# Sbte/RAILS

Measured on AMD Instinct MI355X. Metric: RAILS iterations/sec (+ A*V SpMM HBM GB/s in roofline), m=1M rows/GPU, k=128, fp64, higher is better.
Workload: dtype f64

## Files before the change

### include/rails_hip.h

```cpp
#ifndef RAILS_HIP_H
#define RAILS_HIP_H

#include <stddef.h>
#include <stdint.h>

#ifdef __cplusplus
extern "C" {
#endif

#define RAILS_OK 0
#define RAILS_EINVAL -1
#define RAILS_EHIP -2
#define RAILS_ENOMEM -3
#define RAILS_ELAPACK -4
#define RAILS_ECOMM -5
#define RAILS_ENODEV -6

typedef struct rails_ctx rails_ctx;
typedef struct rails_csr rails_csr;
typedef struct rails_panel rails_panel;

const char *rails_last_error(void);
const char *rails_version(void);


int rails_ctx_create(int device, void *stream, rails_ctx **out);
int rails_ctx_destroy(rails_ctx *ctx);
int rails_ctx_sync(rails_ctx *ctx);
void *rails_ctx_stream(rails_ctx *ctx);
int rails_ctx_stats(rails_ctx *ctx, char *buf, int cap);
int rails_ctx_set_meter(rails_ctx *ctx, int on);

int rails_ctx_set_seed(rails_ctx *ctx, uint64_t seed, uint64_t first_stream);
int rails_ctx_rng_state(rails_ctx *ctx, uint64_t *seed, uint64_t *next_stream);

int rails_ctx_set_partition(rails_ctx *ctx, int rank, int nranks, int64_t row0, int64_t m_global);

typedef int (*rails_allreduce_fn)(void *user, double *dev_buf, size_t n, void *stream);
int rails_ctx_set_allreduce(rails_ctx *ctx, rails_allreduce_fn fn, void *user);

#define RAILS_RCCL_ID_BYTES 128
int rails_rccl_unique_id(void *id_out);
int rails_ctx_init_rccl(rails_ctx *ctx, const void *id, int nranks, int rank);
int rails_ctx_set_rccl(rails_ctx *ctx, void *nccl_comm);
int rails_ctx_rccl_size(const rails_ctx *ctx);

typedef int (*rails_halo_fn)(void *user, const double *send_buf, double *recv_buf, int ncols, void *stream);


// ... 56 lines not shown
int rails_panel_reserve(rails_ctx *ctx, rails_panel *P, int capacity);

int rails_panel_upload(rails_ctx *ctx, rails_panel *P, int c0, int nc, const double *host, int64_t ldh);
int rails_panel_download(rails_ctx *ctx, const rails_panel *P, int c0, int nc, double *host, int64_t ldh);

int rails_panel_fill(rails_ctx *ctx, rails_panel *P, int c0, int nc, double value);
int rails_panel_scale(rails_ctx *ctx, rails_panel *P, int c0, int nc, double s);
int rails_panel_copy(rails_ctx *ctx, const rails_panel *X, int xc0, int nc, rails_panel *Y, int yc0);
int rails_panel_axpy(rails_ctx *ctx, double alpha, const rails_panel *X, int xc0, int nc, rails_panel *Y,
                     int yc0);
int rails_panel_random(rails_ctx *ctx, rails_panel *P, int c0, int nc);

int rails_gram(rails_ctx *ctx, const rails_panel *X, int xc0, int a, const rails_panel *Y, int yc0, int b,
               double *C_host, int ldc);

int rails_panel_gemm(rails_ctx *ctx, double alpha, const rails_panel *X, int xc0, int k, const double *C_host,
                     int ldc, int r, double beta, rails_panel *Y, int yc0);

int rails_ctx_enable_library_gemm(rails_ctx *ctx);
int rails_ctx_library_gemm_ready(const rails_ctx *ctx);

int rails_deferred_reserve(rails_ctx *ctx, int nslots, int64_t doubles_per_slot);
int rails_gram_deferred(rails_ctx *ctx, const rails_panel *X, int xc0, int a, const rails_panel *Y, int yc0, int b, int slot);
int rails_panel_gemm_deferred(rails_ctx *ctx, double alpha, const rails_panel *X, int xc0, int k, int slot, int ld, int r, double beta,
                              rails_panel *Y, int yc0);
int rails_chol_inverse_deferred(rails_ctx *ctx, int slot_in, int w, int slot_out);
int rails_update_gram_deferred(rails_ctx *ctx, double alpha, const rails_panel *X, int xc0, int k, const double *C_host, int ldc, int r,
                               rails_panel *Y, int yc0, int r2, int slot);
int rails_deferred_fetch(rails_ctx *ctx, int slot, int64_t n, double *host_out);

int rails_panel_gemm_wide(rails_ctx *ctx, double alpha, const rails_panel *X, int xc0, int k, const double *C_host, int ldc, int r,
                          double beta, rails_panel *Y, int yc0);

int rails_orthogonalize(rails_ctx *ctx, rails_panel *V, int k_old, int w, int method, int *used);
int rails_orthogonalize_deflated(rails_ctx *ctx, rails_panel *V, int k_old, int w, const rails_panel *N, int nc0, int q, int method, int *used);

int rails_resid_lanczos(rails_ctx *ctx, const rails_panel *AV, int avc0, const rails_panel *MV, int mvc0, int k,
                        const double *T_host, int ldt, const rails_panel *B, int bc0, int p, int L,
                        double *H_host, int ldh, int *steps);

int rails_lanczos_start(rails_ctx *ctx, const rails_panel *AV, int avc0, const rails_panel *MV, int mvc0, int k,
                        const rails_panel *B, int bc0, int p, double *sums_host);

int rails_lanczos_vectors(rails_ctx *ctx, const double *S_host, int lds, int w, rails_panel *Out, int oc0);
int rails_lanczos_release(rails_ctx *ctx);

int rails_ctx_reserve_staging(rails_ctx *ctx, size_t bytes);
int rails_timer_start(rails_ctx *ctx);
int rails_timer_stop(rails_ctx *ctx, double *ms);


void rails_sb03md(char dico, char job, char fact, char trans, int n, double *A, int lda, double *X, int ldx,
                  double *scale, int *info);
void rails_sb03md_counts(long *smith, long *schur);
void rails_sb03md_adi_counts(long *extended, long *fresh);
void rails_sb03md_set_pause(int calls);
void rails_dsyev(char jobz, char uplo, int n, double *a, int lda, double *w, int *info);
void rails_dsteqr(char compz, int n, double *d, double *e, double *z, int ldz, double *work, int *info);
void rails_dgemm(char transa, char transb, int m, int n, int k, double alpha, const double *A, int lda, const double *B,
                 int ldb, double beta, double *C, int ldc);
void rails_dtrsm(char side, char uplo, char transa, char diag, int m, int n, double alpha, const double *A, int lda, double *B, int ldb);
void rails_dpotrf(char uplo, int n, double *a, int lda, int *info);
void rails_dpstrf(char uplo, int n, double *a, int lda, int *piv, int *rank, double tol, int *info);
void rails_range_basis(int m, int n, double *a, int lda, double tol, double *q, int ldq, int *rank, int *info);
int rails_host_lapack_init(const char *path);
const char *rails_host_lapack_path(void);

#ifdef __cplusplus
}
#endif
#endif
```

### rails_amd/_lib.py

```python
import ctypes as C
import os

_HERE = os.path.dirname(os.path.abspath(__file__))
LIB_PATH = os.path.join(_HERE, "lib", "librails_hip.so")

_dp = C.POINTER(C.c_double)
_ip = C.POINTER(C.c_int)
_i64p = C.POINTER(C.c_int64)
_i32p = C.POINTER(C.c_int32)
_vp = C.c_void_p

ALLREDUCE_FN = C.CFUNCTYPE(C.c_int, C.c_void_p, C.c_void_p, C.c_size_t, C.c_void_p)
HALO_FN = C.CFUNCTYPE(C.c_int, C.c_void_p, C.c_void_p, C.c_void_p, C.c_int, C.c_void_p)
APPLY_FN = C.CFUNCTYPE(C.c_int, C.c_void_p, C.c_int, C.c_void_p, C.c_int, C.c_int, C.c_void_p, C.c_int)

SIGNATURES = {
    "rails_last_error": (C.c_char_p, []),
    "rails_version": (C.c_char_p, []),
    "rails_ctx_create": (C.c_int, [C.c_int, _vp, C.POINTER(_vp)]),
    "rails_ctx_destroy": (C.c_int, [_vp]),
    "rails_ctx_sync": (C.c_int, [_vp]),
    "rails_ctx_stream": (_vp, [_vp]),
    "rails_ctx_set_meter": (C.c_int, [_vp, C.c_int]),
    "rails_ctx_enable_library_gemm": (C.c_int, [_vp]),
# ... 29 lines not shown
    "rails_sweep_plan_create": (C.c_int, [C.c_int64, C.c_int64, _i64p, _i32p, _dp, _ip, C.POINTER(_vp)]),
    "rails_sweep_plan_destroy": (C.c_int, [_vp]),
    "rails_sweep_plan_info": (C.c_int, [_vp, _i64p, _dp]),
    "rails_sweep_plan_array": (C.c_int, [_vp, C.c_int, C.POINTER(_vp), _i64p]),
    "rails_panel_create": (C.c_int, [_vp, C.c_int64, C.c_int, C.POINTER(_vp)]),
    "rails_panel_destroy": (C.c_int, [_vp]),
    "rails_panel_rows": (C.c_int64, [_vp]),
    "rails_panel_capacity": (C.c_int, [_vp]),
    "rails_panel_ld": (C.c_int, [_vp]),
    "rails_panel_device_ptr": (_vp, [_vp]),
    "rails_panel_reserve": (C.c_int, [_vp, _vp, C.c_int]),
    "rails_panel_upload": (C.c_int, [_vp, _vp, C.c_int, C.c_int, _dp, C.c_int64]),
    "rails_panel_download": (C.c_int, [_vp, _vp, C.c_int, C.c_int, _dp, C.c_int64]),
    "rails_panel_fill": (C.c_int, [_vp, _vp, C.c_int, C.c_int, C.c_double]),
    "rails_panel_scale": (C.c_int, [_vp, _vp, C.c_int, C.c_int, C.c_double]),
    "rails_panel_copy": (C.c_int, [_vp, _vp, C.c_int, C.c_int, _vp, C.c_int]),
    "rails_panel_axpy": (C.c_int, [_vp, C.c_double, _vp, C.c_int, C.c_int, _vp, C.c_int]),
    "rails_sptrsv_create": (C.c_int, [_vp, C.c_int64, _i64p, _i32p, _dp, C.c_int, C.c_int, C.POINTER(_vp)]),
    "rails_sptrsv_destroy": (None, [_vp]),
    "rails_sptrsv_levels": (C.c_int64, [_vp]),
    "rails_sptrsv_solve": (C.c_int, [_vp, _vp, _vp, C.c_int, C.c_int]),
    "rails_panel_permute_rows": (C.c_int, [_vp, _vp, C.c_int, C.c_int, _vp, C.c_int, _vp, C.c_int]),
    "rails_index_upload": (C.c_int, [_vp, _i32p, C.c_int64, C.POINTER(_vp)]),
    "rails_index_free": (None, [_vp, _vp]),
    "rails_lu_create": (C.c_int, [_vp, C.c_int64, _i64p, _i32p, _dp, _i64p, _i32p, _dp, _i32p, _i32p, _i32p, C.c_int64, C.POINTER(_vp)]),
    "rails_lu_destroy": (None, [_vp]),
    "rails_lu_solve": (C.c_int, [_vp, _vp, C.c_int, _vp, C.c_int, C.c_int, _vp, C.c_int]),
    "rails_lu_stats": (C.c_int, [_vp, _i64p, C.c_int]),
    "rails_csr_create_lu": (C.c_int, [_vp, _vp, C.POINTER(_vp)]),
    "rails_panel_random": (C.c_int, [_vp, _vp, C.c_int, C.c_int]),
    "rails_gram": (C.c_int, [_vp, _vp, C.c_int, C.c_int, _vp, C.c_int, C.c_int, _dp, C.c_int]),
    "rails_panel_gemm": (C.c_int, [_vp, C.c_double, _vp, C.c_int, C.c_int, _dp, C.c_int, C.c_int, C.c_double, _vp, C.c_int]),
    "rails_panel_gemm_wide": (C.c_int, [_vp, C.c_double, _vp, C.c_int, C.c_int, _dp, C.c_int, C.c_int, C.c_double, _vp, C.c_int]),
    "rails_orthogonalize": (C.c_int, [_vp, _vp, C.c_int, C.c_int, C.c_int, _ip]),
    "rails_orthogonalize_deflated": (C.c_int, [_vp, _vp, C.c_int, C.c_int, _vp, C.c_int, C.c_int, C.c_int, _ip]),
    "rails_resid_lanczos": (C.c_int, [_vp, _vp, C.c_int, _vp, C.c_int, C.c_int, _dp, C.c_int, _vp, C.c_int, C.c_int, C.c_int,
                                      _dp, C.c_int, _ip]),
    "rails_lanczos_start": (C.c_int, [_vp, _vp, C.c_int, _vp, C.c_int, C.c_int, _vp, C.c_int, C.c_int, _dp]),
    "rails_lanczos_vectors": (C.c_int, [_vp, _dp, C.c_int, C.c_int, _vp, C.c_int]),
    "rails_lanczos_release": (C.c_int, [_vp]),
    "rails_timer_start": (C.c_int, [_vp]),
    "rails_timer_stop": (C.c_int, [_vp, _dp]),
    "rails_sb03md": (None, [C.c_char, C.c_char, C.c_char, C.c_char, C.c_int, _dp, C.c_int, _dp, C.c_int, _dp, _ip]),
    "rails_dsyev": (None, [C.c_char, C.c_char, C.c_int, _dp, C.c_int, _dp, _ip]),
    "rails_dsteqr": (None, [C.c_char, C.c_int, _dp, _dp, _dp, C.c_int, _dp, _ip]),
    "rails_ctx_reserve_staging": (C.c_int, [_vp, C.c_size_t]),
    "rails_sb03md_set_pause": (None, [C.c_int]),
    "rails_sb03md_counts": (None, [C.POINTER(C.c_long), C.POINTER(C.c_long)]),
    "rails_sb03md_adi_counts": (None, [C.POINTER(C.c_long), C.POINTER(C.c_long)]),
    "rails_dtrsm": (None, [C.c_char, C.c_char, C.c_char, C.c_char, C.c_int, C.c_int, C.c_double, _dp, C.c_int, _dp, C.c_int]),
    "rails_dgemm": (None, [C.c_char, C.c_char, C.c_int, C.c_int, C.c_int, C.c_double, _dp, C.c_int, _dp, C.c_int, C.c_double, _dp, C.c_int]),
    "rails_dpotrf": (None, [C.c_char, C.c_int, _dp, C.c_int, _ip]),
    "rails_dpstrf": (None, [C.c_char, C.c_int, _dp, C.c_int, _ip, _ip, C.c_double, _ip]),
    "rails_range_basis": (None, [C.c_int, C.c_int, _dp, C.c_int, C.c_double, _dp, C.c_int, _ip, _ip]),
    "rails_host_lapack_init": (C.c_int, [C.c_char_p]),
    "rails_host_lapack_path": (C.c_char_p, []),
}

_lib = None


class RailsError(RuntimeError):
    pass


def load():
    global _lib
    if _lib is not None:
        return _lib
    if not os.path.exists(LIB_PATH):
        raise RailsError(
            "rails_amd: %s is missing -- build it with `python -c 'import __graft_entry__ as g; g.build()'` "
            "or `make -C rails_amd/csrc`; there is no CPU fallback" % LIB_PATH)
    lib = C.CDLL(LIB_PATH, mode=C.RTLD_GLOBAL)
    for name, (res, args) in SIGNATURES.items():
        fn = getattr(lib, name)
        fn.restype = res
        fn.argtypes = args
    try:
        from ._solver_sigs import bind as _bind_solver
        _bind_solver(lib)
    except ImportError:
        pass
    _lib = lib
    return lib


# ... 5 lines not shown
```

### rails_amd/csrc/host_numerics.cpp

```cpp
#include <dlfcn.h>

#include <algorithm>
#include <atomic>
#include <chrono>
#include <utility>
#include <cmath>
#include <cstdio>
#include <cstdlib>
#include <cstring>
#include <mutex>
#include <string>
#include <vector>

#include "rails_hip.h"

void rails_set_error(const char *fmt, ...);

namespace {

extern "C" {
typedef int (*lp_select2)(const double *, const double *);
typedef void (*lp_dsyev)(const char *, const char *, const int *, double *, const int *, double *, double *, const int *, int *);
typedef void (*lp_dsyevd)(const char *, const char *, const int *, double *, const int *, double *, double *, const int *, int *, const int *, int *);
typedef void (*lp_dsteqr)(const char *, const int *, double *, double *, double *, const int *, double *, int *);
// ... 315 lines not shown
    *rank = 0;
    if (rails_host_lapack_init(nullptr) != RAILS_OK || !g_lp.dgeqp3 || !g_lp.dorgqr) {
        *info = -100;
        return;
    }
    if (m <= 0 || n <= 0) {
        *info = 0;
        return;
    }
    const int kmin = m < n ? m : n;
    std::vector<int> jpvt((size_t)n, 0);
    std::vector<double> tau((size_t)kmin);
    double wq = 0.0;
    int lwork = -1;
    g_lp.dgeqp3(&m, &n, a, &lda, jpvt.data(), tau.data(), &wq, &lwork, info);
    if (*info != 0) return;
    lwork = (int)wq + 1;
    std::vector<double> work((size_t)lwork);
    g_lp.dgeqp3(&m, &n, a, &lda, jpvt.data(), tau.data(), work.data(), &lwork, info);
    if (*info != 0) return;
    const double r11 = std::fabs(a[0]);
    int r = 0;
    while (r < kmin && std::fabs(a[r + (size_t)r * lda]) > tol * r11 && r11 > 0.0) ++r;
    *rank = r;
    if (r == 0) return;
    for (int j = 0; j < r; ++j)
        for (int i = 0; i < m; ++i) q[i + (size_t)j * ldq] = a[i + (size_t)j * lda];
    lwork = -1;
    g_lp.dorgqr(&m, &r, &r, q, &ldq, tau.data(), &wq, &lwork, info);
    if (*info != 0) return;
    lwork = (int)wq + 1;
    work.resize((size_t)lwork);
    g_lp.dorgqr(&m, &r, &r, q, &ldq, tau.data(), work.data(), &lwork, info);
}

static int &sb03md_smith_pause()
{
    static thread_local int pause = 0;
    return pause;
}
static int &sb03md_factored_pause()
{
    static thread_local int pause = 0;
    return pause;
}
extern "C" void rails_sb03md_set_pause(int calls) { sb03md_smith_pause() = sb03md_factored_pause() = calls > 0 ? calls : 0; }
static std::atomic<long> g_sb03md_smith{0}, g_sb03md_schur{0};
extern "C" void rails_sb03md_counts(long *smith, long *schur)
{
    if (smith) *smith = g_sb03md_smith.load();
    if (schur) *schur = g_sb03md_schur.load();
}

static bool smith_lyapunov(bool tr, int n, const double *A, int lda, double *X, int ldx)
{
    if (!g_lp.dgetrf || !g_lp.dgetrs) return false;
    const size_t nn = (size_t)n * n;
    std::vector<double> M(nn), S(nn), Ak(nn), Y(nn), T1(nn), T2(nn), C(nn);
    double trace = 0.0;
    for (int j = 0; j < n; ++j) {
        for (int i = 0; i < n; ++i) {
            M[i + (size_t)j * n] = tr ? A[i + (size_t)j * lda] : A[j + (size_t)i * lda];
            C[i + (size_t)j * n] = 0.5 * (X[i + (size_t)j * ldx] + X[j + (size_t)i * ldx]);
        }
        trace += A[j + (size_t)j * lda];
    }
// ... 569 lines not shown
```

### rails_amd/csrc/solver_capi.cpp

```cpp
#include <cmath>
#include <cstdio>
#include <cstring>
#include <map>
#include <string>
#include <vector>

#include <exception>
#include <new>

#include "rails/HipSolverOps.hpp"
#include "rails/SubspaceSolverOps.hpp"
#include "rails_solver.h"

void rails_set_error(const char *fmt, ...);

namespace
{

class ParameterList
{
    std::map<std::string, double> params_;

public:
    template <typename T>
// ... 206 lines not shown
    rails::HipSolver::Projection proj;
    const bool pair = rails::HipSolver::parse_projection(s->params.get("Projection method", 1.0), proj) && proj.pair;
    const int kmax = std::max(restart > 0 ? restart : 100, 1) + (pair ? 2 : 1) * expand + 100;
    auto basis = std::make_shared<rails::SubspaceBasis>(s->ctx, s->m_local, s->m_global, 2 * kmax + p + 128);
    if (restart > 0 || s->params.get("Restart iterations", 20) > 0) basis->preallocate_compress_panel();
    rails::SubspaceMultiVector Bc = rails::SubspaceMultiVector::Absorb(basis, s->B);
    rails::SubspaceOperator Ac(s->A, basis);
    rails::SubspaceOperator Mc(s->mass ? s->M : s->A, basis);
    rails::SubspaceSolver solver(Ac, Bc, Mc);
    if (s->has_inv) solver.set_inverse(rails::SubspaceOperator(s->Ainv, basis));
    if (s->null_q > 0) solver.set_nullspace(rails::SubspaceMultiVector::Absorb(basis, s->N));
    int prc = solver.set_parameters(s->params);
    if (prc != 0) return prc + 100;
    solver.set_verbose(s->verbose);
    solver.set_max_trips(s->max_trips);
    solver.use_mass_matrix(s->mass);
    solver.use_mass_orthogonalisation(s->ortho_m);
    if (s->trip_fn) solver.set_trip_callback([s](int trip) { s->trip_fn(s->trip_user, trip); });
    solver.set_failure_check([basis]() { return basis->failed; });
    rails::SubspaceMultiVector Vc(basis, 1);
    if (s->have_V0) {
        Vc = rails::SubspaceMultiVector::Absorb(basis, s->V);
        Vc.set_orthogonalized(Vc.N());
    }
    int rc = solver.solve(Vc, s->T);
    s->null_rank = solver.nullspace_rank();
    if (rc == -2) return rc;
    s->V = Vc.materialise();
    s->V.set_orthogonalized(s->V.N());
    s->sub_trips = solver.trips();
    s->sub_hist = solver.residual_history();
    s->sub_profile = solver.profile();
    char buf[1536];
    snprintf(buf, sizeof(buf), "{\"dim\": %d, \"absorb\": %ld, \"absorb_columns\": %ld, \"one_by_one\": %ld, \"dropped\": %ld, \"compress\": %ld, \"materialise\": %ld, \"prefetched_random\": %ld, \"second_rounds\": %ld, \"delicate_blocks\": %ld, \"reprojected_blocks\": %ld, \"overlapped_blocks\": %ld, \"replaced_columns\": %ld, \"verified\": %d, \"verify_representation\": %.3e, \"verify_orthonormality\": %.3e, \"seconds\": {\"materialise\": %.4f, \"absorb\": %.4f, \"compress_qr\": %.4f, \"compress_rotate\": %.4f, "
             "\"compress_coefficients\": %.4f}}",
             basis->dim, basis->n_absorb, basis->n_absorb_cols, basis->n_single, basis->n_dropped, basis->n_compress, basis->n_materialise, basis->n_prefetched, basis->n_second_round, basis->n_delicate, basis->n_reprojected, basis->n_overlapped, basis->n_replaced, basis->verify ? 1 : 0, basis->verify_repr, basis->verify_orth,
             basis->t_materialise, basis->t_absorb, basis->t_qr, basis->t_rotate, basis->t_recoef);
    s->sub_stats = buf;
    if (basis->failed) {
        rails_set_error("coordinate-space back end: a device operation failed (%s)", rails_last_error());
        return -1000;
    }
    return rc;
}

extern "C" int rails_solver_solve(rails_solver *s, int *code, int *k)
{
    if (!s) return RAILS_EINVAL;
    const bool restart_from_solution = s->params.get("Restart from solution", 0.0) != 0.0;
    s->last_was_subspace = s->subspace && (s->have_V0 || !restart_from_solution);
    {
        rails::HipSolver::Projection proj;
        const double method = s->params.get("Projection method", 1.0);
        if (!rails::HipSolver::parse_projection(method, proj)) {
            rails_set_error("rails_solver_solve: 'Projection method' %g is none of 1, 1.1, 1.2, 1.3, 2.1, 2.2, 2.3", method);
            return RAILS_EINVAL;
        }
        if (proj.uses_inverse() && !s->has_inv) {
            rails_set_error("rails_solver_solve: 'Projection method' %g needs an inverse (rails_solver_set_inverse)", method);
            return RAILS_EINVAL;
        }
    }
    rails::clear_sticky_error();
    int rc;
    try {
        if (s->last_was_subspace) {
            rc = solve_in_coordinates(s);
            if (rc == -1000) return RAILS_EHIP;
        } else {
// ... 118 lines not shown
```

### rails_amd/include/rails/SubspaceWrappers.hpp

```cpp
#ifndef RAILS_SUBSPACEWRAPPERS_HPP
#define RAILS_SUBSPACEWRAPPERS_HPP

#include <algorithm>
#include <atomic>
#include <chrono>
#include <cmath>
#include <cstdlib>
#include <cstring>
#include <iostream>
#include <memory>
#include <vector>

#include "rails/HipWrappers.hpp"

namespace rails
{

struct CoefStore {
    std::vector<double> c;
    int ld = 0, ncap = 0;
    bool in_basis = true;
    CoefStore(int ld_, int ncap_, bool in_basis_) : c((size_t)std::max(ld_, 1) * std::max(ncap_, 1), 0.0), ld(ld_), ncap(std::max(ncap_, 1)), in_basis(in_basis_) {}
    double *col(int j) { return c.data() + (size_t)j * ld; }
    const double *col(int j) const { return c.data() + (size_t)j * ld; }
};

class SubspaceBasis
{
public:
    rails_ctx *ctx;
    int64_t m_local, m_global;
    HipMultiVectorWrapper P, P2;
    int dim = 0;
    int row_cap;
    std::vector<std::weak_ptr<CoefStore>> live;
    long n_absorb = 0, n_absorb_cols = 0, n_single = 0, n_compress = 0, n_materialise = 0, n_dropped = 0, n_prefetched = 0, n_second_round = 0, n_delicate = 0, n_reprojected = 0;
    bool failed = false;
    long n_replaced = 0;
    double t_materialise = 0, t_absorb = 0, t_qr = 0, t_rotate = 0, t_recoef = 0;
    bool profile_sync = getenv("RAILS_SUBSPACE_PROFILE") != nullptr;
    bool trace = getenv("RAILS_SUBSPACE_TRACE") != nullptr;
    double reorth_survival = getenv("RAILS_SUBSPACE_REORTH") ? atof(getenv("RAILS_SUBSPACE_REORTH")) : 0.5;
    double slow_ms = getenv("RAILS_SUBSPACE_SLOW_MS") ? atof(getenv("RAILS_SUBSPACE_SLOW_MS")) : 0.0;
    struct Tick {
        SubspaceBasis *b;
        double *acc;
        const char *what;
        std::chrono::steady_clock::time_point t0;
        Tick(SubspaceBasis *bb, double *a, const char *w = "") : b(bb), acc(a), what(w)
        {
            if (b->profile_sync) rails_ctx_sync(b->ctx);
            t0 = std::chrono::steady_clock::now();
        }
        ~Tick()
        {
            if (b->profile_sync) rails_ctx_sync(b->ctx);
            const double dt = std::chrono::duration<double>(std::chrono::steady_clock::now() - t0).count();
            *acc += dt;
            if (b->slow_ms > 0.0 && dt * 1e3 > b->slow_ms)
                std::cerr << "[subspace] " << what << ": " << dt * 1e3 << " ms (dim " << b->dim << ", absorbs so far " << b->n_absorb << ")" << std::endl;
        }
    };
    std::shared_ptr<CoefStore> cached_random;
    bool cached_valid = false;
    bool prefetch_random = true;

    bool overlap = !(getenv("RAILS_SUBSPACE_OVERLAP") && atoi(getenv("RAILS_SUBSPACE_OVERLAP")) == 0);
    double overlap_min_survival = 1e-4;
    long n_overlapped = 0;
    struct Pending {
        bool active = false;
        int dim0 = 0, w = 0, w2 = 0;
        std::vector<double> Rfp;
        std::vector<double> g0diag;
    } pending;
    enum { SLOT_C2 = 0, SLOT_G = 1, SLOT_M1 = 2, SLOT_G2 = 3, SLOT_M2 = 4, N_SLOTS = 5 };

    SubspaceBasis(rails_ctx *c, int64_t ml, int64_t mg, int rows) : ctx(c), m_local(ml), m_global(mg), P(ml, std::max(rows, 16), c), row_cap(std::max(rows, 16))
    {
        P.set_global_rows(mg);
        P.resize(0);
    }

    void preallocate_compress_panel()
    {
        const size_t cap = (size_t)P.capacity();
        hip_ok(rails_ctx_reserve_staging(ctx, cap * cap / 2 * sizeof(double)), "rails_ctx_reserve_staging");
        if (P2.N() >= 0 && P2.capacity() >= P.capacity()) return;
        P2 = HipMultiVectorWrapper(m_local, P.capacity(), ctx);
        P2.set_global_rows(m_global);
        const int kw = std::min(256, (int)P.capacity());
        if (kw >= 64 && rails_ctx_library_gemm_ready(ctx)) {
            std::vector<double> Z((size_t)kw * kw, 0.0);
            const int keep = P.N();
            P.resize(kw);
            P2.resize(kw);
            hip_ok(rails_panel_fill(ctx, P.panel(), keep, kw - keep, 0.0), "rails_panel_fill");
            hip_ok(rails_panel_gemm_wide(ctx, 1.0, P.panel(), 0, kw, Z.data(), kw, kw, 0.0, P2.panel(), 0), "rails_panel_gemm_wide");
            P.resize(keep);
        }
        P2.resize(0);
    }

    std::shared_ptr<CoefStore> new_store(int ncap, bool in_basis, int rows = 0)
    {
        auto s = std::make_shared<CoefStore>(in_basis ? row_cap : rows, ncap, in_basis);
        if (in_basis) live.push_back(s);
        return s;
    }

    void ensure_rows(int need)
    {
        if (need <= row_cap) return;
        int ncap = std::max(need + 64, row_cap + row_cap / 2);
        for (auto &w : live)
            if (auto s = w.lock()) {
                std::vector<double> nc((size_t)ncap * s->ncap, 0.0);
                for (int j = 0; j < s->ncap; ++j) memcpy(nc.data() + (size_t)j * ncap, s->col(j), sizeof(double) * dim);
                s->c.swap(nc);
                s->ld = ncap;
// ... 249 lines not shown
                ncols += s->ncap;
            }
        live.swap(still);
        if (dim == 0 || ncols == 0) return;
        std::vector<double> Call((size_t)dim * ncols);
        int c0 = 0;
        for (auto &s : stores)
            for (int j = 0; j < s->ncap; ++j) {
                const double *cj = s->col(j);
                bool nz = false;
                for (int i = 0; i < dim && !nz; ++i) nz = cj[i] != 0.0;
                if (!nz) continue;
                memcpy(Call.data() + (size_t)c0 * dim, cj, sizeof(double) * dim);
                ++c0;
            }
        ncols = c0;
        if (trace) {
            std::cerr << "compress: dim " << dim << ", " << stores.size() << " live stores, columns in use:";
            for (auto &st : stores) {
                int used = 0;
                for (int j = 0; j < st->ncap; ++j) {
                    const double *cj = st->col(j);
                    for (int i = 0; i < dim; ++i)
                        if (cj[i] != 0.0) {
                            ++used;
                            break;
                        }
                }
                std::cerr << " " << used << "/" << st->ncap;
            }
            std::cerr << " -> " << ncols << " columns" << std::endl;
        }
        if (ncols == 0) return;
        std::vector<double> Q((size_t)dim * std::min(dim, ncols));
        int rank = 0, info = 0;
        {
            Tick tick(this, &t_qr, "compress: pivoted QR");
            rails_range_basis(dim, ncols, Call.data(), dim, 1e-14, Q.data(), dim, &rank, &info);
        }
        if (info != 0 || rank <= 0 || rank >= dim - 8) return;
        if (P2.N() < 0 || P2.capacity() < rank + 64) {
            P2 = HipMultiVectorWrapper(m_local, rank + 128, ctx);
            P2.set_global_rows(m_global);
        }
        P2.resize(rank);
        {
            Tick rot(this, &t_rotate, "compress: rotation");
            if (!hip_ok(rails_panel_gemm_wide(ctx, 1.0, P.panel(), 0, dim, Q.data(), dim, rank, 0.0, P2.panel(), 0), "rails_panel_gemm_wide")) {
                failed = true;
                return;
            }
        }
        Tick tick(this, &t_recoef, "compress: coefficients");
        for (auto &s : stores) {
            int used = 0;
            for (int j = s->ncap - 1; j >= 0 && !used; --j) {
                const double *cj = s->col(j);
                for (int i = 0; i < dim; ++i)
                    if (cj[i] != 0.0) {
                        used = j + 1;
                        break;
                    }
            }
            if (used == 0) continue;
            std::vector<double> nc((size_t)rank * used);
            rails_dgemm('T', 'N', rank, used, dim, 1.0, Q.data(), dim, s->c.data(), s->ld, 0.0, nc.data(), rank);
            for (int j = 0; j < used; ++j) {
                memcpy(s->col(j), nc.data() + (size_t)j * rank, sizeof(double) * rank);
                std::fill(s->col(j) + rank, s->col(j) + dim, 0.0);
            }
        }
        std::swap(P, P2);
        dim = rank;
        n_compress++;
    }

    bool start_overlapped(int w, int w2, double *coef, std::vector<double> const &CG, std::vector<double> const &G0)
    {
        const int ld = row_cap, dw = dim + w;
        std::vector<double> Gp((size_t)w * w), d(w);
        for (int j = 0; j < w; ++j)
            for (int i = 0; i <= j; ++i) {
                double s = 0.0;
                for (int l = 0; l < dim; ++l) s += CG[l + (size_t)i * dw] * CG[l + (size_t)j * dw];
                Gp[i + (size_t)j * w] = Gp[j + (size_t)i * w] = G0[i + (size_t)j * w] - s;
            }
        for (int j = 0; j < w; ++j) {
            if (!(Gp[j + (size_t)j * w] > 1e-8 * G0[j + (size_t)j * w]) || !(Gp[j + (size_t)j * w] > 0.0)) return false;
            d[j] = std::sqrt(Gp[j + (size_t)j * w]);
        }
        std::vector<double> R1((size_t)w * w);
        for (int b = 0; b < w; ++b)
            for (int a = 0; a < w; ++a) R1[a + (size_t)b * w] = Gp[a + (size_t)b * w] / (d[a] * d[b]);
        int info = 0;
        rails_dpotrf('U', w, R1.data(), w, &info);
        if (info != 0) return false;
        for (int a = 0; a < w; ++a)
            if (!(R1[a + (size_t)a * w] > 1e-2)) return false;
        if (!hip_ok(rails_deferred_reserve(ctx, N_SLOTS, (int64_t)(P.capacity() + 64) * (w <= 32 ? 32 : 48)), "rails_deferred_reserve")) return false;
        rails_panel *pp = P.panel();
        bool ok = true;
        if (w2 > 0) {
            ok = ok && hip_ok(rails_update_gram_deferred(ctx, -1.0, pp, 0, dim, CG.data(), dw, w, pp, dim, w2, SLOT_C2), "rails_update_gram_deferred");
            ok = ok && hip_ok(rails_panel_gemm_deferred(ctx, -1.0, pp, 0, dim, SLOT_C2, dim, w2, 1.0, pp, dim), "rails_panel_gemm_deferred");
        } else
            ok = ok && hip_ok(rails_panel_gemm(ctx, -1.0, pp, 0, dim, CG.data(), dw, w, 1.0, pp, dim), "rails_panel_gemm");
        ok = ok && hip_ok(rails_gram_deferred(ctx, pp, dim, w, pp, dim, w, SLOT_G), "rails_gram_deferred");
// ... 629 lines not shown
```

Before: 228.6.

## Compress subspace basis in place with compact block Householder reflector

When the basis is compressed, the full dense rotation into a second panel (dim x rank GEMM) is replaced. The new path computes a compact WY block reflector from the pivoted QR of the coefficients, then applies it in place with a new MFMA-based HIP kernel that touches only d reflector columns. This drops the second panel allocation and cuts the flop and traffic count when few reflectors are needed. The cost is extra host-side LAPACK work, a new hand-written kernel using LDS-DMA inline assembly, and a warm-up launch that pre-compiles it.

```diff
diff --git a/include/rails_hip.h b/include/rails_hip.h
--- a/include/rails_hip.h
+++ b/include/rails_hip.h
@@ -15,6 +15,7 @@
 #define RAILS_ELAPACK -4
 #define RAILS_ECOMM -5
 #define RAILS_ENODEV -6
+#define RAILS_ESHAPE -7
 
 typedef struct rails_ctx rails_ctx;
 typedef struct rails_csr rails_csr;
@@ -137,6 +138,10 @@
 int rails_panel_gemm_wide(rails_ctx *ctx, double alpha, const rails_panel *X, int xc0, int k, const double *C_host, int ldc, int r,
                           double beta, rails_panel *Y, int yc0);
 
+int rails_panel_reflect(rails_ctx *ctx, rails_panel *P, int c0, int k, const double *Y_host, int ldy, int d, const double *S_host, int lds,
+                        int r);
+int rails_panel_reflect_supported(int k, int d, int r);
+
 int rails_orthogonalize(rails_ctx *ctx, rails_panel *V, int k_old, int w, int method, int *used);
 int rails_orthogonalize_deflated(rails_ctx *ctx, rails_panel *V, int k_old, int w, const rails_panel *N, int nc0, int q, int method, int *used);
 
@@ -168,6 +173,8 @@
 void rails_dpotrf(char uplo, int n, double *a, int lda, int *info);
 void rails_dpstrf(char uplo, int n, double *a, int lda, int *piv, int *rank, double tol, int *info);
 void rails_range_basis(int m, int n, double *a, int lda, double tol, double *q, int ldq, int *rank, int *info);
+void rails_range_reflector(int m, int n, double *a, int lda, double tol, int dmax, double *Y, int ldy, double *T, int ldt, double *S, int lds,
+                           int *rank, int *d, int *info);
 int rails_host_lapack_init(const char *path);
 const char *rails_host_lapack_path(void);
 
diff --git a/rails_amd/_lib.py b/rails_amd/_lib.py
--- a/rails_amd/_lib.py
+++ b/rails_amd/_lib.py
@@ -85,6 +85,8 @@
     "rails_gram": (C.c_int, [_vp, _vp, C.c_int, C.c_int, _vp, C.c_int, C.c_int, _dp, C.c_int]),
     "rails_panel_gemm": (C.c_int, [_vp, C.c_double, _vp, C.c_int, C.c_int, _dp, C.c_int, C.c_int, C.c_double, _vp, C.c_int]),
     "rails_panel_gemm_wide": (C.c_int, [_vp, C.c_double, _vp, C.c_int, C.c_int, _dp, C.c_int, C.c_int, C.c_double, _vp, C.c_int]),
+    "rails_panel_reflect": (C.c_int, [_vp, _vp, C.c_int, C.c_int, _dp, C.c_int, C.c_int, _dp, C.c_int, C.c_int]),
+    "rails_panel_reflect_supported": (C.c_int, [C.c_int, C.c_int, C.c_int]),
     "rails_orthogonalize": (C.c_int, [_vp, _vp, C.c_int, C.c_int, C.c_int, _ip]),
     "rails_orthogonalize_deflated": (C.c_int, [_vp, _vp, C.c_int, C.c_int, _vp, C.c_int, C.c_int, C.c_int, _ip]),
     "rails_resid_lanczos": (C.c_int, [_vp, _vp, C.c_int, _vp, C.c_int, C.c_int, _dp, C.c_int, _vp, C.c_int, C.c_int, C.c_int,
@@ -106,6 +108,7 @@
     "rails_dpotrf": (None, [C.c_char, C.c_int, _dp, C.c_int, _ip]),
     "rails_dpstrf": (None, [C.c_char, C.c_int, _dp, C.c_int, _ip, _ip, C.c_double, _ip]),
     "rails_range_basis": (None, [C.c_int, C.c_int, _dp, C.c_int, C.c_double, _dp, C.c_int, _ip, _ip]),
+    "rails_range_reflector": (None, [C.c_int, C.c_int, _dp, C.c_int, C.c_double, C.c_int, _dp, C.c_int, _dp, C.c_int, _dp, C.c_int, _ip, _ip, _ip]),
     "rails_host_lapack_init": (C.c_int, [C.c_char_p]),
     "rails_host_lapack_path": (C.c_char_p, []),
 }
diff --git a/rails_amd/csrc/host_numerics.cpp b/rails_amd/csrc/host_numerics.cpp
--- a/rails_amd/csrc/host_numerics.cpp
+++ b/rails_amd/csrc/host_numerics.cpp
@@ -371,6 +371,111 @@
     lwork = (int)wq + 1;
     work.resize((size_t)lwork);
     g_lp.dorgqr(&m, &r, &r, q, &ldq, tau.data(), work.data(), &lwork, info);
+}
+
+extern "C" void rails_range_reflector(int m, int n, double *a, int lda, double tol, int dmax, double *Y, int ldy, double *T, int ldt, double *S, int lds, int *rank,
+                                      int *d_out, int *info)
+{
+    *rank = 0;
+    *d_out = 0;
+    if (rails_host_lapack_init(nullptr) != RAILS_OK || !g_lp.dgeqp3 || !g_lp.dorgqr) {
+        *info = -100;
+        return;
+    }
+    *info = 0;
+    if (m <= 0 || n <= 0) return;
+    const int kmin = m < n ? m : n;
+    std::vector<int> jpvt((size_t)n, 0);
+    std::vector<double> tau((size_t)kmin);
+    double wq = 0.0;
+    int lwork = -1;
+    g_lp.dgeqp3(&m, &n, a, &lda, jpvt.data(), tau.data(), &wq, &lwork, info);
+    if (*info != 0) return;
+    lwork = (int)wq + 1;
+    std::vector<double> work((size_t)lwork);
+    g_lp.dgeqp3(&m, &n, a, &lda, jpvt.data(), tau.data(), work.data(), &lwork, info);
+    if (*info != 0) return;
+    const double r11 = std::fabs(a[0]);
+    int r = 0;
+    while (r < kmin && std::fabs(a[r + (size_t)r * lda]) > tol * r11 && r11 > 0.0) ++r;
+    const int d = m - r;
+    *rank = r;
+    *d_out = d;
+    if (d == 0 || r == 0) return;
+    if (d > dmax) {
+        *info = 1;
+        return;
+    }
+    std::vector<double> q((size_t)m * m, 0.0);
+    for (int j = 0; j < r; ++j)
+        for (int i = j + 1; i < m; ++i) q[i + (size_t)j * m] = a[i + (size_t)j * lda];
+    lwork = -1;
+    g_lp.dorgqr(&m, &m, &r, q.data(), &m, tau.data(), &wq, &lwork, info);
+    if (*info != 0) return;
+    lwork = (int)wq + 1;
+    work.resize((size_t)lwork);
+    g_lp.dorgqr(&m, &m, &r, q.data(), &m, tau.data(), work.data(), &lwork, info);
+    if (*info != 0) return;
+    std::vector<double> M((size_t)m * d), tq((size_t)d), w((size_t)d);
+    for (int j = 0; j < d; ++j)
+        for (int i = 0; i < m; ++i) M[i + (size_t)j * m] = q[(m - 1 - i) + (size_t)(m - 1 - j) * m];
+    for (int j = 0; j < d; ++j) {
+        double *x = M.data() + (size_t)j * m;
+        double s2 = 0.0;
+        for (int i = j + 1; i < m; ++i) s2 += x[i] * x[i];
+        const double alpha = x[j];
+        if (s2 == 0.0) {
+            tq[j] = 0.0;
+            continue;
+        }
+        const double beta = -std::copysign(std::sqrt(alpha * alpha + s2), alpha);
+        tq[j] = (beta - alpha) / beta;
+        const double sc = 1.0 / (alpha - beta);
+        for (int i = j + 1; i < m; ++i) x[i] *= sc;
+        x[j] = beta;
+        for (int c = j + 1; c < d; ++c) {
+            double *y = M.data() + (size_t)c * m;
+            double dot = y[j];
+            for (int i = j + 1; i < m; ++i) dot += x[i] * y[i];
+            dot *= tq[j];
+            y[j] -= dot;
+            for (int i = j + 1; i < m; ++i) y[i] -= dot * x[i];
+        }
+    }
+    for (int j = 0; j < d; ++j) {
+        double *y = Y + (size_t)j * ldy;
+        for (int i = 0; i < m; ++i) {
+            const int iv = m - 1 - i;
+            y[i] = iv < j ? 0.0 : (iv == j ? 1.0 : M[iv + (size_t)j * m]);
+        }
+    }
+    for (int j = 0; j < d; ++j) {
+        double *tj = T + (size_t)j * ldt;
+        const double *yj = Y + (size_t)j * ldy;
+        for (int i = 0; i < j; ++i) {
+            const double *yi = Y + (size_t)i * ldy;
+            double dot = 0.0;
+            for (int l = 0; l < m - j; ++l) dot += yi[l] * yj[l];
+            w[i] = dot;
+        }
+        for (int i = 0; i < j; ++i) {
+            double acc = 0.0;
+            for (int l = i; l < j; ++l) acc += T[i + (size_t)l * ldt] * w[l];
+            tj[i] = -tq[j] * acc;
+        }
+        tj[j] = tq[j];
+        for (int i = j + 1; i < d; ++i) tj[i] = 0.0;
+    }
+    for (int c = 0; c < r; ++c) {
+        double *sc = S + (size_t)c * lds;
+        for (int i = 0; i < d; ++i) sc[i] = 0.0;
+        for (int l = 0; l < d; ++l) {
+            const double ycl = Y[c + (size_t)l * ldy];
+            if (ycl == 0.0) continue;
+            const double *tl = T + (size_t)l * ldt;
+            for (int i = 0; i <= l; ++i) sc[i] += tl[i] * ycl;
+        }
+    }
 }
 
 static int &sb03md_smith_pause()
diff --git a/rails_amd/csrc/reflect.hip b/rails_amd/csrc/reflect.hip
--- /dev/null
+++ b/rails_amd/csrc/reflect.hip
@@ -0,0 +1,230 @@
+#include "rails_internal.h"
+
+#include <algorithm>
+
+namespace {
+
+typedef double v4f64 __attribute__((ext_vector_type(4)));
+typedef double v2f64 __attribute__((ext_vector_type(2)));
+
+__device__ __forceinline__ v4f64 mfma_f64(double a, double b, v4f64 c)
+{
+    return __builtin_amdgcn_mfma_f64_16x16x4f64(a, b, c, 0, 0, 0);
+}
+
+__global__ void k_pack_rows(const double *__restrict__ C, int k, int r, int kpad, int RL, double *__restrict__ out)
+{
+    const int64_t n = (int64_t)kpad * RL;
+    for (int64_t q = (int64_t)blockIdx.x * blockDim.x + threadIdx.x; q < n; q += (int64_t)gridDim.x * blockDim.x) {
+        const int kl = (int)(q / RL), j = (int)(q % RL);
+        out[q] = (kl < k && j < r) ? C[kl + (int64_t)j * k] : 0.0;
+    }
+}
+
+template <int TR, int TZ>
+__global__ __launch_bounds__(512) void k_panel_reflect(double *X, int ldx, int k, const double *__restrict__ Yt , const double *__restrict__ St ,
+                                                       int r, int64_t m, int vec_ok)
+{
+    constexpr int KC = 32, RL = 16 * TR + 4, RLZ = 16 * TZ + 4, CHS = KC * RL * 8, CHZ = KC * RLZ * 8, TWL = 18, TW_B = 16 * TWL * 8;
+    static_assert(CHS % 1024 == 0 && CHZ % 1024 == 0, "whole LDS-DMA pieces per chunk");
+    static_assert(TZ % 2 == 0 && TZ <= TR && 8 * TW_B <= CHS, "Z chunks fit the S buffers; the turn-around fits the second one");
+    extern __shared__ double Cs[];
+    const int lane = threadIdx.x & 63;
+    const int wave = __builtin_amdgcn_readfirstlane((int)(threadIdx.x >> 6));
+    const int li = lane & 15, kk = lane >> 4;
+    const int64_t r0 = ((int64_t)blockIdx.x * 8 + wave) * 16;
+    const int64_t myrow = r0 + li;
+    const bool rowok = myrow < m;
+    const uint32_t lds_base = (uint32_t)(uintptr_t)(__attribute__((address_space(3))) unsigned char *)Cs;
+    const uint32_t lane16 = (uint32_t)lane * 16u;
+    auto stage = [&](const double *packed, int chunk, int bytes) {
+        const char *src = reinterpret_cast<const char *>(packed) + (size_t)chunk * bytes;
+        const uint32_t dst = lds_base + (uint32_t)((chunk & 1) * bytes);
+        for (int p = wave; p < bytes / 1024; p += 8) {
+            uint32_t keep;
+            asm volatile("s_mov_b32 %0, m0\n\ts_mov_b32 m0, %3\n\ts_nop 0\n\tglobal_load_lds_dwordx4 %1, %2\n\ts_mov_b32 m0, %0"
+                         : "=&s"(keep) : "v"(lane16), "s"(src + (size_t)p * 1024), "s"(dst + (uint32_t)(p * 1024)) : "memory");
+        }
+    };
+    const double *xrow = X + (rowok ? myrow : m - 1) * ldx;
+    auto fetch = [&](int kcol, double *xs) {
+        if (vec_ok && kcol + 4 <= k) {
+            v2f64 t0 = *reinterpret_cast<const v2f64 *>(xrow + kcol);
+            v2f64 t1 = *reinterpret_cast<const v2f64 *>(xrow + kcol + 2);
+            xs[0] = t0.x;
+            xs[1] = t0.y;
+            xs[2] = t1.x;
+            xs[3] = t1.y;
+        } else {
+#pragma unroll
+            for (int s = 0; s < 4; ++s) xs[s] = (kcol + s < k) ? xrow[kcol + s] : 0.0;
+        }
+    };
+    double zr[4 * TZ];
+    {
+        v4f64 zacc[TZ];
+#pragma unroll
+        for (int t = 0; t < TZ; ++t) zacc[t] = (v4f64){0.0, 0.0, 0.0, 0.0};
+        const int nchunks = (k + KC - 1) / KC;
+        double xa[4], xb[4];
+        stage(Yt, 0, CHZ);
+        fetch(4 * kk, xa);
+        fetch(16 + 4 * kk, xb);
+        asm volatile("s_waitcnt vmcnt(0)" : : : "memory");
+        __builtin_amdgcn_s_barrier();
+        for (int ci = 0; ci < nchunks; ++ci) {
+            if (ci + 1 < nchunks) stage(Yt, ci + 1, CHZ);
+            double xc[4], xd[4];
+            fetch((ci + 1) * KC + 4 * kk, xc);
+            fetch((ci + 1) * KC + 16 + 4 * kk, xd);
+            const double *cb = Cs + (size_t)(ci & 1) * (KC * RLZ);
+#pragma unroll
+            for (int s = 0; s < 4; ++s) {
+                const double *crow = &cb[(4 * kk + s) * RLZ + li];
+#pragma unroll
+                for (int t = 0; t < TZ; ++t) zacc[t] = mfma_f64(xa[s], crow[16 * t], zacc[t]);
+            }
+#pragma unroll
+            for (int s = 0; s < 4; ++s) {
+                const double *crow = &cb[(16 + 4 * kk + s) * RLZ + li];
+#pragma unroll
+                for (int t = 0; t < TZ; ++t) zacc[t] = mfma_f64(xb[s], crow[16 * t], zacc[t]);
+            }
+#pragma unroll
+            for (int s = 0; s < 4; ++s) {
+                xa[s] = xc[s];
+                xb[s] = xd[s];
+            }
+            asm volatile("s_waitcnt vmcnt(0) lgkmcnt(0)" : : : "memory");
+            __builtin_amdgcn_s_barrier();
+        }
+        stage(St, 0, CHS);
+        double *Tw = Cs + (CHS + wave * TW_B) / 8;
+#pragma unroll
+        for (int t = 0; t < TZ; ++t) {
+#pragma unroll
+            for (int v = 0; v < 4; ++v) Tw[(kk + 4 * v) * TWL + li] = zacc[t][v];
+            __builtin_amdgcn_fence(__ATOMIC_RELEASE, "wavefront");
+            __builtin_amdgcn_wave_barrier();
+            __builtin_amdgcn_fence(__ATOMIC_ACQUIRE, "wavefront");
+            const v2f64 a0 = *reinterpret_cast<const v2f64 *>(&Tw[li * TWL + 4 * kk]);
+            const v2f64 a1 = *reinterpret_cast<const v2f64 *>(&Tw[li * TWL + 4 * kk + 2]);
+            zr[4 * t + 0] = -a0.x;
+            zr[4 * t + 1] = -a0.y;
+            zr[4 * t + 2] = -a1.x;
+            zr[4 * t + 3] = -a1.y;
+            __builtin_amdgcn_fence(__ATOMIC_RELEASE, "wavefront");
+            __builtin_amdgcn_wave_barrier();
+        }
+    }
+    v4f64 acc[TR];
+#pragma unroll
+    for (int t = 0; t < TR; ++t) {
+        const int j = 16 * t + li;
+#pragma unroll
+        for (int v = 0; v < 4; ++v) {
+            const int64_t row = r0 + kk + 4 * v;
+            acc[t][v] = X[(row < m ? row : m - 1) * ldx + (j < r ? j : 0)];
+        }
+    }
+    asm volatile("s_waitcnt vmcnt(0) lgkmcnt(0)" : : : "memory");
+    __builtin_amdgcn_s_barrier();
+#pragma unroll
+    for (int ci = 0; ci < TZ / 2; ++ci) {
+        if (ci + 1 < TZ / 2) stage(St, ci + 1, CHS);
+        const double *cb = Cs + (size_t)(ci & 1) * (KC * RL);
+#pragma unroll
+        for (int s = 0; s < 4; ++s) {
+            const double *crow = &cb[(4 * kk + s) * RL + li];
+#pragma unroll
+            for (int t = 0; t < TR; ++t) acc[t] = mfma_f64(zr[8 * ci + s], crow[16 * t], acc[t]);
+        }
+#pragma unroll
+        for (int s = 0; s < 4; ++s) {
+            const double *crow = &cb[(16 + 4 * kk + s) * RL + li];
+#pragma unroll
+            for (int t = 0; t < TR; ++t) acc[t] = mfma_f64(zr[8 * ci + 4 + s], crow[16 * t], acc[t]);
+        }
+        if (ci + 1 < TZ / 2) {
+            asm volatile("s_waitcnt vmcnt(0) lgkmcnt(0)" : : : "memory");
+            __builtin_amdgcn_s_barrier();
+        }
+    }
+#pragma unroll
+    for (int t = 0; t < TR; ++t) {
+        const int j = 16 * t + li;
+        if (j >= r) continue;
+#pragma unroll
+        for (int v = 0; v < 4; ++v) {
+            const int64_t row = r0 + kk + 4 * v;
+            if (row < m) X[row * ldx + j] = acc[t][v];
+        }
+    }
+}
+
+template <int TR, int TZ>
+int launch_reflect(rails_ctx *c, double *X, int ldx, int k, const double *yt, const double *st, int r, int64_t m, int vec_ok)
+{
+    const size_t lds = (size_t)2 * 32 * (16 * TR + 4) * sizeof(double);
+    RAILS_HIP_CHECK(hipFuncSetAttribute((const void *)k_panel_reflect<TR, TZ>, hipFuncAttributeMaxDynamicSharedMemorySize, (int)lds));
+    RAILS_LAUNCH((k_panel_reflect<TR, TZ>), dim3((unsigned)((m + 127) / 128)), dim3(512), lds, c->stream, X, ldx, k, yt, st, r, m, vec_ok);
+    return RAILS_OK;
+}
+
+template <int TR>
+int launch_reflect_tz(rails_ctx *c, int tz, double *X, int ldx, int k, const double *yt, const double *st, int r, int64_t m, int vec_ok)
+{
+    switch (tz) {
+    case 2: return launch_reflect<TR, 2>(c, X, ldx, k, yt, st, r, m, vec_ok);
+    case 4: return launch_reflect<TR, 4>(c, X, ldx, k, yt, st, r, m, vec_ok);
+    case 6: return launch_reflect<TR, 6>(c, X, ldx, k, yt, st, r, m, vec_ok);
+    default:
+        if constexpr (TR >= 8) return launch_reflect<TR, 8>(c, X, ldx, k, yt, st, r, m, vec_ok);
+        return RAILS_EINVAL;
+    }
+}
+
+}
+
+extern "C" int rails_panel_reflect_supported(int k, int d, int r) { return k >= 1 && d >= 1 && d <= 128 && r >= 1 && r <= 288 && r <= k ? 1 : 0; }
+
+extern "C" int rails_panel_reflect(rails_ctx *c, rails_panel *P, int c0, int k, const double *Y_host, int ldy, int d, const double *S_host, int lds, int r)
+{
+    if (c) hipSetDevice(c->device);
+    rails_slow_guard slow__(c, "rails_panel_reflect", k, d);
+    RAILS_REQUIRE(c && P && Y_host && S_host, "rails_panel_reflect: null argument");
+    RAILS_REQUIRE(k >= 1 && d >= 1 && r >= 1 && r <= k && c0 >= 0 && c0 + k <= P->cap, "rails_panel_reflect: window [%d,%d), %d output columns, capacity %d", c0, c0 + k, r,
+                  P->cap);
+    RAILS_REQUIRE(ldy >= k && lds >= d, "rails_panel_reflect: bad leading dimensions (ldy %d < %d or lds %d < %d)", ldy, k, lds, d);
+    if (!rails_panel_reflect_supported(k, d, r)) {
+        rails_set_error("rails_panel_reflect: d = %d > 128 reflectors or r = %d > 288 output columns", d, r);
+        return RAILS_ESHAPE;
+    }
+    if (P->m == 0) return RAILS_OK;
+    const int tz = (d + 31) / 32 * 2, trz = std::max(std::max(6, (r + 31) / 32 * 2), tz);
+    const int kpad = (k + 31) / 32 * 32, RL = 16 * trz + 4, RLZ = 16 * tz + 4;
+    const size_t ny = (size_t)k * d, ns = (size_t)d * r, nyt = (size_t)kpad * RLZ, nst = (size_t)16 * tz * RL;
+    RAILS_TRY(rails_small_reserve(c, (ny + ns) * sizeof(double)));
+    RAILS_TRY(rails_ws_reserve(c, (nyt + nst) * sizeof(double)));
+    RAILS_TRY(rails_pinned_begin_write(c, (ny + ns) * sizeof(double)));
+    for (int j = 0; j < d; ++j) memcpy(c->pinned + (size_t)j * k, Y_host + (size_t)j * ldy, sizeof(double) * k);
+    for (int j = 0; j < r; ++j) memcpy(c->pinned + ny + (size_t)j * d, S_host + (size_t)j * lds, sizeof(double) * d);
+    RAILS_HIP_CHECK(hipMemcpyAsync(c->small, c->pinned, (ny + ns) * sizeof(double), hipMemcpyHostToDevice, c->stream));
+    RAILS_TRY(rails_pinned_end_write(c));
+    double *yt = c->ws, *st = c->ws + nyt;
+    RAILS_LAUNCH(k_pack_rows, dim3((unsigned)std::min<size_t>(512, (nyt + 255) / 256)), dim3(256), 0, c->stream, c->small, k, d, kpad, RLZ, yt);
+    RAILS_LAUNCH(k_pack_rows, dim3((unsigned)std::min<size_t>(512, (nst + 255) / 256)), dim3(256), 0, c->stream, c->small + ny, d, r, 16 * tz, RL, st);
+    double *X = P->d + c0;
+    const int vec_ok = ((((uintptr_t)X) & 15) == 0 && (P->ld % 2) == 0) ? 1 : 0;
+    switch (trz) {
+    case 6: RAILS_TRY((launch_reflect_tz<6>(c, tz, X, P->ld, k, yt, st, r, P->m, vec_ok))); break;
+    case 8: RAILS_TRY((launch_reflect_tz<8>(c, tz, X, P->ld, k, yt, st, r, P->m, vec_ok))); break;
+    case 10: RAILS_TRY((launch_reflect_tz<10>(c, tz, X, P->ld, k, yt, st, r, P->m, vec_ok))); break;
+    case 12: RAILS_TRY((launch_reflect_tz<12>(c, tz, X, P->ld, k, yt, st, r, P->m, vec_ok))); break;
+    case 14: RAILS_TRY((launch_reflect_tz<14>(c, tz, X, P->ld, k, yt, st, r, P->m, vec_ok))); break;
+    case 16: RAILS_TRY((launch_reflect_tz<16>(c, tz, X, P->ld, k, yt, st, r, P->m, vec_ok))); break;
+    default: RAILS_TRY((launch_reflect_tz<18>(c, tz, X, P->ld, k, yt, st, r, P->m, vec_ok))); break;
+    }
+    RAILS_HIP_CHECK(hipGetLastError());
+    return RAILS_OK;
+}
diff --git a/rails_amd/csrc/solver_capi.cpp b/rails_amd/csrc/solver_capi.cpp
--- a/rails_amd/csrc/solver_capi.cpp
+++ b/rails_amd/csrc/solver_capi.cpp
@@ -262,9 +262,9 @@
     s->sub_hist = solver.residual_history();
     s->sub_profile = solver.profile();
     char buf[1536];
-    snprintf(buf, sizeof(buf), "{\"dim\": %d, \"absorb\": %ld, \"absorb_columns\": %ld, \"one_by_one\": %ld, \"dropped\": %ld, \"compress\": %ld, \"materialise\": %ld, \"prefetched_random\": %ld, \"second_rounds\": %ld, \"delicate_blocks\": %ld, \"reprojected_blocks\": %ld, \"overlapped_blocks\": %ld, \"replaced_columns\": %ld, \"verified\": %d, \"verify_representation\": %.3e, \"verify_orthonormality\": %.3e, \"seconds\": {\"materialise\": %.4f, \"absorb\": %.4f, \"compress_qr\": %.4f, \"compress_rotate\": %.4f, "
+    snprintf(buf, sizeof(buf), "{\"dim\": %d, \"absorb\": %ld, \"absorb_columns\": %ld, \"one_by_one\": %ld, \"dropped\": %ld, \"compress\": %ld, \"compress_reflect\": %ld, \"materialise\": %ld, \"prefetched_random\": %ld, \"second_rounds\": %ld, \"delicate_blocks\": %ld, \"reprojected_blocks\": %ld, \"overlapped_blocks\": %ld, \"replaced_columns\": %ld, \"verified\": %d, \"verify_representation\": %.3e, \"verify_orthonormality\": %.3e, \"seconds\": {\"materialise\": %.4f, \"absorb\": %.4f, \"compress_qr\": %.4f, \"compress_rotate\": %.4f, "
              "\"compress_coefficients\": %.4f}}",
-             basis->dim, basis->n_absorb, basis->n_absorb_cols, basis->n_single, basis->n_dropped, basis->n_compress, basis->n_materialise, basis->n_prefetched, basis->n_second_round, basis->n_delicate, basis->n_reprojected, basis->n_overlapped, basis->n_replaced, basis->verify ? 1 : 0, basis->verify_repr, basis->verify_orth,
+             basis->dim, basis->n_absorb, basis->n_absorb_cols, basis->n_single, basis->n_dropped, basis->n_compress, basis->n_reflect, basis->n_materialise, basis->n_prefetched, basis->n_second_round, basis->n_delicate, basis->n_reprojected, basis->n_overlapped, basis->n_replaced, basis->verify ? 1 : 0, basis->verify_repr, basis->verify_orth,
              basis->t_materialise, basis->t_absorb, basis->t_qr, basis->t_rotate, basis->t_recoef);
     s->sub_stats = buf;
     if (basis->failed) {
diff --git a/rails_amd/include/rails/SubspaceWrappers.hpp b/rails_amd/include/rails/SubspaceWrappers.hpp
--- a/rails_amd/include/rails/SubspaceWrappers.hpp
+++ b/rails_amd/include/rails/SubspaceWrappers.hpp
@@ -35,6 +35,11 @@
     int row_cap;
     std::vector<std::weak_ptr<CoefStore>> live;
     long n_absorb = 0, n_absorb_cols = 0, n_single = 0, n_compress = 0, n_materialise = 0, n_dropped = 0, n_prefetched = 0, n_second_round = 0, n_delicate = 0, n_reprojected = 0;
+    long n_reflect = 0;
+    bool reflect = !(getenv("RAILS_SUBSPACE_REFLECT") && atoi(getenv("RAILS_SUBSPACE_REFLECT")) == 0);
+    enum { REFLECT_DMAX = 128 };
+    int64_t reflect_min_rows = getenv("RAILS_SUBSPACE_REFLECT_MIN_ROWS") ? atoll(getenv("RAILS_SUBSPACE_REFLECT_MIN_ROWS")) : 65536;
+    bool use_reflector() const { return reflect && m_global >= reflect_min_rows; }
     bool failed = false;
     long n_replaced = 0;
     double t_materialise = 0, t_absorb = 0, t_qr = 0, t_rotate = 0, t_recoef = 0;
@@ -86,6 +91,17 @@
     {
         const size_t cap = (size_t)P.capacity();
         hip_ok(rails_ctx_reserve_staging(ctx, cap * cap / 2 * sizeof(double)), "rails_ctx_reserve_staging");
+        if (use_reflector()) {
+            const int kw = std::min(352, (int)P.capacity()), dw = 64, keep = P.N();
+            if (kw >= 2 * dw && keep <= kw - dw) {
+                std::vector<double> Z((size_t)kw * dw, 0.0);
+                P.resize(kw);
+                hip_ok(rails_panel_fill(ctx, P.panel(), keep, kw - keep, 0.0), "rails_panel_fill");
+                hip_ok(rails_panel_reflect(ctx, P.panel(), 0, kw, Z.data(), kw, dw, Z.data(), dw, kw - dw), "rails_panel_reflect");
+                P.resize(keep);
+            }
+            return;
+        }
         if (P2.N() >= 0 && P2.capacity() >= P.capacity()) return;
         P2 = HipMultiVectorWrapper(m_local, P.capacity(), ctx);
         P2.set_global_rows(m_global);
@@ -401,13 +417,52 @@
             std::cerr << " -> " << ncols << " columns" << std::endl;
         }
         if (ncols == 0) return;
+        int rank = 0, info = 0;
+        if (use_reflector()) {
+            const int dmax = std::min<int>(REFLECT_DMAX, dim);
+            std::vector<double> Cw(Call.begin(), Call.begin() + (size_t)dim * ncols);
+            std::vector<double> Y((size_t)dim * dmax), T((size_t)dmax * dmax), S((size_t)dmax * dim);
+            int d = 0;
+            {
+                Tick tick(this, &t_qr, "compress: pivoted QR");
+                rails_range_reflector(dim, ncols, Cw.data(), dim, 1e-14, dmax, Y.data(), dim, T.data(), dmax, S.data(), dmax, &rank, &d, &info);
+            }
+            if ((info != 0 && info != 1) || rank <= 0 || rank >= dim - 8) return;
+            if (info == 0 && (long)d * (dim + rank) < (long)dim * rank && rails_panel_reflect_supported(dim, d, rank)) {
+                if (trace) std::cerr << "compress: block reflector, dim " << dim << " -> rank " << rank << " (" << d << " reflectors)" << std::endl;
+                {
+                    Tick rot(this, &t_rotate, "compress: rotation");
+                    if (!hip_ok(rails_panel_reflect(ctx, P.panel(), 0, dim, Y.data(), dim, d, S.data(), dmax, rank), "rails_panel_reflect")) {
+                        failed = true;
+                        return;
+                    }
+                }
+                Tick tick(this, &t_recoef, "compress: coefficients");
+                std::vector<double> W1, W2;
+                for (auto &s : stores) {
+                    const int used = used_columns(*s);
+                    if (used == 0) continue;
+                    W1.resize((size_t)d * used);
+                    W2.resize((size_t)d * used);
+                    rails_dgemm('T', 'N', d, used, dim, 1.0, Y.data(), dim, s->c.data(), s->ld, 0.0, W1.data(), d);
+                    rails_dgemm('T', 'N', d, used, d, 1.0, T.data(), dmax, W1.data(), d, 0.0, W2.data(), d);
+                    rails_dgemm('N', 'N', dim, used, d, -1.0, Y.data(), dim, W2.data(), d, 1.0, s->c.data(), s->ld);
+                    for (int j = 0; j < used; ++j) std::fill(s->col(j) + rank, s->col(j) + dim, 0.0);
+                }
+                P.resize(rank);
+                dim = rank;
+                n_compress++;
+                n_reflect++;
+                return;
+            }
+        }
         std::vector<double> Q((size_t)dim * std::min(dim, ncols));
-        int rank = 0, info = 0;
         {
             Tick tick(this, &t_qr, "compress: pivoted QR");
             rails_range_basis(dim, ncols, Call.data(), dim, 1e-14, Q.data(), dim, &rank, &info);
         }
         if (info != 0 || rank <= 0 || rank >= dim - 8) return;
+        if (trace) std::cerr << "compress: dense rotation, dim " << dim << " -> rank " << rank << std::endl;
         if (P2.N() < 0 || P2.capacity() < rank + 64) {
             P2 = HipMultiVectorWrapper(m_local, rank + 128, ctx);
             P2.set_global_rows(m_global);
@@ -422,15 +477,7 @@
         }
         Tick tick(this, &t_recoef, "compress: coefficients");
         for (auto &s : stores) {
-            int used = 0;
-            for (int j = s->ncap - 1; j >= 0 && !used; --j) {
-                const double *cj = s->col(j);
-                for (int i = 0; i < dim; ++i)
-                    if (cj[i] != 0.0) {
-                        used = j + 1;
-                        break;
-                    }
-            }
+            const int used = used_columns(*s);
             if (used == 0) continue;
             std::vector<double> nc((size_t)rank * used);
             rails_dgemm('T', 'N', rank, used, dim, 1.0, Q.data(), dim, s->c.data(), s->ld, 0.0, nc.data(), rank);
@@ -442,6 +489,16 @@
         std::swap(P, P2);
         dim = rank;
         n_compress++;
+    }
+
+    int used_columns(const CoefStore &s) const
+    {
+        for (int j = s.ncap - 1; j >= 0; --j) {
+            const double *cj = s.col(j);
+            for (int i = 0; i < dim; ++i)
+                if (cj[i] != 0.0) return j + 1;
+        }
+        return 0;
     }
 
     bool start_overlapped(int w, int w2, double *coef, std::vector<double> const &CG, std::vector<double> const &G0)
```

Result: slower. 224.5 (median of 2 runs) (-1.8%).
